# hansungkim98122/IGT-MPC-INT

Measured on NVIDIA B200. Metric: converged MPC solves/sec, higher is better.
Workload: dtype f64

## Files before the change

### igt_mpc_int_b200/csrc/igt_abi.cu

```cuda
#include <cuda_runtime.h>
#include <cstdio>
#include <cstdlib>
#include <cstring>
#include <string>
#include <vector>
#include <new>
#include <mutex>

#include "../../include/igt_mpc.h"
#include "solver_core.cuh"
#include "params_host.hpp"
#include "mlp_tc.cuh"

using namespace igt;

#ifndef SOLVE_BLOCK
#define SOLVE_BLOCK 256
#endif
#define SLOTS_PER_SM SOLVE_BLOCK

constexpr int N_CSLOTS = 8;
__constant__ DevParams<float> c_Pf[N_CSLOTS];
__constant__ DevParams<double> c_Pd[N_CSLOTS];
static_assert(N_CSLOTS * (sizeof(DevParams<float>) + sizeof(DevParams<double>)) <= 60 * 1024, "constant memory budget");

template <> struct igt::ConstP<float> { static __device__ __forceinline__ const DevParams<float> &get(int s) { return c_Pf[s]; } };
template <> struct igt::ConstP<double> { static __device__ __forceinline__ const DevParams<double> &get(int s) { return c_Pd[s]; } };
#include "episode.cuh"

template <typename T, bool OBCA>
__global__ void __launch_bounds__(128) guess_kernel(ProbIO io, long B, double *guess, int cs)
{
    long p = (long)blockIdx.x * blockDim.x + threadIdx.x;
    if (p >= B) return;
    if (io.u_init && (!io.warm || io.warm[p])) return;
    const DevParams<T> &P = ConstP<T>::get(cs);
    Solver<T, Ws<T, 32, OBCA>> sv(P);
    sv.compute_guess(io, p, guess + p * P.N * 2);
}

#ifndef IGT_RSTG
#define IGT_RSTG 1
#endif
template <typename T, bool TC, bool OBCA, bool COOP = false, bool BANK = false>
__global__ void __launch_bounds__(SOLVE_BLOCK, 1) solve_kernel(typename std::conditional<BANK, ProbIONet<T>, ProbIO>::type io, T *ws, long n_slots, long B, Sched sc,
                                                               const double *guess, T *mlp_scratch, int mlp_width,
                                                               MlpTcWeights wt, int quota, int cs)
{
    extern __shared__ __align__(16) uint8_t dyn_smem[];
    long slot = (long)blockIdx.x * blockDim.x + threadIdx.x;
    const DevParams<T> &P = ConstP<T>::get(cs);
    MlpTcCtx tc;
    if (TC) mlp_tc_setup(tc, dyn_smem, wt);
    constexpr bool RSTG = IGT_RSTG && !TC && !COOP;
    solve_persistent<T, TC, 32, OBCA, COOP, RSTG, BANK>(P, io, ws, slot, B, sc, guess,
                            mlp_scratch ? mlp_scratch + slot * 12 * (long)mlp_width : nullptr, mlp_width, &tc, quota, cs, dyn_smem,
                            RSTG ? dyn_smem + (COOP ? mlp_coop_smem_bytes<T>(SOLVE_BLOCK) : 0) : nullptr);
    if (TC) mlp_tc_teardown(tc);
}

template <typename T, bool OBCA>
__global__ void __launch_bounds__(SOLVE_BLOCK, 1) solve_small_kernel(ProbIO io, long B, Sched sc, const double *guess, int cs)
{
    extern __shared__ __align__(16) uint8_t dyn_smem[];
    const DevParams<T> &P = ConstP<T>::get(cs);
    solve_persistent<T, false, 1, OBCA>(P, io, reinterpret_cast<T *>(dyn_smem), 0, B, sc, guess, (T *)nullptr, 0, nullptr, 1, cs);
}

__global__ void __launch_bounds__(128) rollout_kernel(int B, const float *__restrict__ z0,
                                                      const float *__restrict__ U,
                                                      const float *__restrict__ curv_, float *__restrict__ Z,
                                                      float *__restrict__ A, float *__restrict__ Bm, int cs)
{
    int p = blockIdx.x * blockDim.x + threadIdx.x;
    if (p >= B) return;
    const DevParams<float> &P = c_Pf[cs];
    const int N = P.N;
    float z[NZ], comp[NZ], curv[3] = { curv_[3 * p], curv_[3 * p + 1], curv_[3 * p + 2] };
#pragma unroll
    for (int i = 0; i < NZ; i++) { z[i] = z0[(long)p * NZ + i]; comp[i] = 0.f; Z[(long)p * (N + 1) * NZ + i] = z[i]; }
    const float h = P.h;
    for (int k = 0; k < N; k++) {
        float u[2] = { U[((long)p * N + k) * 2], U[((long)p * N + k) * 2 + 1] };
        if (A) {
            float zn[NZ], Sc[NSENS], S[NZ][NSEED];
            rk4_step_sens(P, z, u, curv, zn, Sc);
            expand_sens(P, Sc, S);
            float *Ak = A + ((long)p * N + k) * NZ * NZ, *Bk = Bm + ((long)p * N + k) * NZ * 2;
#pragma unroll
            for (int i = 0; i < NZ; i++) {
#pragma unroll
                for (int j = 0; j < NZ; j++) Ak[i * NZ + j] = (i == j && j < 3) ? 1.f : 0.f;
                Ak[i * NZ + IEY] = S[i][0]; Ak[i * NZ + IEPSI] = S[i][1]; Ak[i * NZ + IV] = S[i][2]; Ak[i * NZ + IPSI] = S[i][3];
                Bk[i * 2] = S[i][4]; Bk[i * 2 + 1] = S[i][5];
            }
        }
        const StepK<float> c = step_setup(P, z, u, curv);
        const double b0d = curv[0], b1d = curv[1];
        auto Kof = [&](double sd) { return (sd >= b0d ? curv[2] : 0.f) - (sd >= b1d ? curv[2] : 0.f); };
        for (int it = 0; it < P.n_rk; it++) {
            Deriv<float> k1, k2, k3, k4;
            RhsJac<float> J;
            const float hh = 0.5f * h;
            const double sd = (double)z[IS] - (double)comp[IS];
            stage_deriv<float, false, true>(c, z[IS], z[IEY], z[IEPSI], z[IV], z[IPSI], k1, J, Kof(sd));
            stage_deriv<float, false, true>(c, z[IS] + hh * k1.s, z[IEY] + hh * k1.ey, z[IEPSI] + hh * k1.ep, z[IV] + hh * u[0],
                                            z[IPSI] + hh * k1.ps, k2, J, Kof(sd + (double)hh * (double)k1.s));
            stage_deriv<float, false, true>(c, z[IS] + hh * k2.s, z[IEY] + hh * k2.ey, z[IEPSI] + hh * k2.ep, z[IV] + hh * u[0],
                                            z[IPSI] + hh * k2.ps, k3, J, Kof(sd + (double)hh * (double)k2.s));
            stage_deriv<float, false, true>(c, z[IS] + h * k3.s, z[IEY] + h * k3.ey, z[IEPSI] + h * k3.ep, z[IV] + h * u[0],
                                            z[IPSI] + hh * k3.ps, k4, J, Kof(sd + (double)h * (double)k3.s));
            float inc[NZ];
            inc[IX] = h / 6.f * (k1.x + 2.f * k2.x + 2.f * k3.x + k4.x);
            inc[IY] = h / 6.f * (k1.y + 2.f * k2.y + 2.f * k3.y + k4.y);
            inc[IS] = h / 6.f * (k1.s + 2.f * k2.s + 2.f * k3.s + k4.s);
            inc[IEY] = h / 6.f * (k1.ey + 2.f * k2.ey + 2.f * k3.ey + k4.ey);
            inc[IEPSI] = h / 6.f * (k1.ep + 2.f * k2.ep + 2.f * k3.ep + k4.ep);
            inc[IV] = h * u[0];
            inc[IPSI] = h / 6.f * (k1.ps + 2.f * k2.ps + 2.f * k3.ps + k4.ps);
// ... 112 lines not shown
                                                      const MlpNet<double> *nets)
{
    long p = (long)blockIdx.x * blockDim.x + threadIdx.x;
    if (p >= B) return;
    const DevParams<double> &P = c_Pd[cs];
    TermVal<double> t;
    double cx[4] = { ctx[4 * p], ctx[4 * p + 1], ctx[4 * p + 2], ctx[4 * p + 3] };
    double *sc = scratch + p * 12 * (long)width;
    if (BANK) mlp_eval_thread_net(nets[net_idx[p]], sN[p], vN[p], cx, sc, sc + 6 * width, width, t, true);
    else mlp_eval_thread(P, sN[p], vN[p], cx, sc, sc + 6 * width, width, t, true);
    out[6 * p] = t.V; out[6 * p + 1] = t.gs; out[6 * p + 2] = t.gv; out[6 * p + 3] = t.Hss; out[6 * p + 4] = t.Hsv; out[6 * p + 5] = t.Hvv;
}

template <bool BANK>
__global__ void __launch_bounds__(256, 1) mlp_coop_kernel(long B, const double *sN, const double *vN, const double *ctx,
                                                          double *out, int cs, const int *net_idx, const MlpNet<double> *nets)
{
    extern __shared__ __align__(16) uint8_t dyn_smem[];
    const DevParams<double> &P = c_Pd[cs];
    for (long base = (long)blockIdx.x * 256; base < B; base += (long)gridDim.x * 256) {
        const long p = base + threadIdx.x;
        const bool valid = p < B;
        double cx[4] = { 0, 0, 0, 0 }, o[6], s = 0, v = 0;
        int net = 0;
        if (valid) { s = sN[p]; v = vN[p]; for (int i = 0; i < 4; i++) cx[i] = ctx[4 * p + i]; if (BANK) net = net_idx[p]; }
        if (BANK) mlp_coop_eval_bank(nets, dyn_smem, valid, net, s, v, cx, o);
        else mlp_coop_eval(P, dyn_smem, valid, s, v, cx, o);
        if (valid) for (int i = 0; i < 6; i++) out[6 * p + i] = o[i];
    }
}

template <typename T>
__global__ void __launch_bounds__(256) fma_peak_kernel(T *out, int iters)
{
    T a0 = T(threadIdx.x) * T(1e-3), a1 = a0 + T(1), a2 = a0 + T(2), a3 = a0 + T(3);
    T a4 = a0 + T(4), a5 = a0 + T(5), a6 = a0 + T(6), a7 = a0 + T(7);
    const T m = T(0.999999), c = T(1e-6);
    for (int i = 0; i < iters; i++) {
        a0 = a0 * m + c; a1 = a1 * m + c; a2 = a2 * m + c; a3 = a3 * m + c;
        a4 = a4 * m + c; a5 = a5 * m + c; a6 = a6 * m + c; a7 = a7 * m + c;
    }
    out[(long)blockIdx.x * blockDim.x + threadIdx.x] = a0 + a1 + a2 + a3 + a4 + a5 + a6 + a7;
}

struct igt_handle {
    igt_params prm;
    DevParams<float> Pf;
    DevParams<double> Pd;
    bool has_mlp = false;
    MlpTcWeights tc = {};
    int use_tc = 0;
    bool coop_ok = false;
    int use_small = 1;
    int mlp_width = 0;
    std::vector<void *> mlp_bufs[MAX_MLP_NETS];
    MlpNet<double> netd[MAX_MLP_NETS] = {};
    MlpNet<float> netf[MAX_MLP_NETS] = {};
    int net_width[MAX_MLP_NETS] = {};
    void *bank = nullptr;
    void *ws = nullptr; size_t ws_bytes = 0;
    void *mlp_scratch = nullptr; size_t mlp_scratch_bytes = 0;
    void *stage = nullptr; size_t stage_bytes = 0;
    void *guess = nullptr; size_t guess_bytes = 0;
    void *episode = nullptr; size_t episode_bytes = 0;
    int n_sm = 0;
    long long launches = 0;
    std::string err;
    int device = 0;
    std::mutex mu;
    cudaStream_t hstream = nullptr;
    void *pin = nullptr; size_t pin_bytes = 0;
    cudaEvent_t last_use = nullptr;
    cudaStream_t last_stream = nullptr;
    bool used = false;
    unsigned long long version[2] = { 1, 1 };
    int cslot[2] = { -1, -1 };
};

struct CSlot { const igt_handle *owner = nullptr; unsigned long long version = 0; cudaEvent_t ev = nullptr; };
constexpr int MAX_DEV = 16;
static std::mutex g_slot_mu;
static CSlot g_slots[MAX_DEV][2][N_CSLOTS];
static unsigned g_slot_rr[MAX_DEV][2];

static std::string g_create_err;
static_assert(IGT_MAX_MLP_NETS == MAX_MLP_NETS, "bank size");

#define CK(call)                                                                                   \
    do {                                                                                           \
        cudaError_t _e = (call);                                                                   \
        if (_e != cudaSuccess) {                                                                   \
            h->err = std::string(#call) + ": " + cudaGetErrorString(_e);                           \
            return IGT_ECUDA;                                                                      \
        }                                                                                          \
    } while (0)

static int grow(igt_handle *h, void **buf, size_t *have, size_t need, cudaStream_t st)
{
    if (*have >= need) return IGT_OK;
    if (*buf) { CK(cudaFreeAsync(*buf, st)); *buf = nullptr; *have = 0; }
    CK(cudaMallocAsync(buf, need, st));
    *have = need;
    return IGT_OK;
}

static int begin_call(igt_handle *h, cudaStream_t st)
// ... 314 lines not shown
    const bool f64 = h->prm.precision == IGT_PREC_F64, obca = obs_psi != nullptr;
    if (obca && !f64) { h->err = "igt_solve: the OBCA collision rows (obs_psi) need precision f64"; return IGT_EINVAL; }
    if (B == 0) return IGT_OK;
    int rc = begin_call(h, st), cs = 0;
    if (rc) return rc;
    WsLayout L; L.init(h->prm.N, h->prm.n_cinf, obca ? NGE_OBCA : NGE, obca ? NHE_OBCA : NHE);
    size_t esz = f64 ? 8 : 4;
    const size_t small_smem = (size_t)L.total * esz;
    const bool small = h->use_small && !nn_ctx && B <= h->n_sm && small_smem <= 200 * 1024;
    const int bs = SOLVE_BLOCK;
    long n_cta = ((long)B + 31) / 32;
    if (n_cta > h->n_sm) n_cta = h->n_sm;
    long per_cta = ((long)B + n_cta - 1) / n_cta;
    int quota = (int)((per_cta + 31) / 32 * 32);
    if (quota > bs) quota = bs;
    long n_slots = n_cta * bs;
    rc = small ? IGT_OK : grow(h, &h->ws, &h->ws_bytes, (size_t)L.total * n_slots * esz, st);
    if (rc) return rc;
    const bool use_tc = nn_ctx && !bank && h->tc.enabled && h->use_tc && !obca;
    const int width = bank ? bank_width(h) : h->mlp_width;
    const bool use_coop = nn_ctx && !use_tc && f64 && (bank ? width <= MLP_COOP_W : h->coop_ok) && !obca;
    if (nn_ctx && !use_tc && !use_coop) {
        rc = grow(h, &h->mlp_scratch, &h->mlp_scratch_bytes, (size_t)12 * width * n_slots * esz, st);
        if (rc) return rc;
    }
    const size_t off_guess = 256;
    rc = grow(h, &h->guess, &h->guess_bytes, off_guess + (size_t)B * h->prm.N * 2 * sizeof(double), st);
    if (rc) return rc;
    char *sb = (char *)h->guess;
    Sched sc;
    sc.counter = (unsigned long long *)sb;
    double *guess = (double *)(sb + off_guess);
    rc = acquire_cslot(h, f64 ? 1 : 0, st, &cs);
    if (rc) return rc;
    CK(cudaMemsetAsync(sb, 0, 256, st));
    ProbIO io = { x0, u_prev, curv, obs_xy, nn_ctx, u_init, x, u, cost, viol, status, iters };
    io.obs_psi = obs_psi;
    io.warm = warm;
    ProbIONet<double> iob;
    static_cast<ProbIO &>(iob) = io;
    iob.net_idx = net_idx;
    iob.nets = (const MlpNet<double> *)h->bank;
    if (!u_init || warm) {
        int gbs = 128, ggs = (B + gbs - 1) / gbs;
        if (obca) guess_kernel<double, true><<<ggs, gbs, 0, st>>>(io, B, guess, cs);
        else if (f64) guess_kernel<double, false><<<ggs, gbs, 0, st>>>(io, B, guess, cs);
        else guess_kernel<float, false><<<ggs, gbs, 0, st>>>(io, B, guess, cs);
        h->launches++;
    }
    int gs = (int)(n_slots / bs);
    if (small) {
        if (obca) {
            CK(cudaFuncSetAttribute(solve_small_kernel<double, true>, cudaFuncAttributeMaxDynamicSharedMemorySize, (int)small_smem));
            solve_small_kernel<double, true><<<B, bs, small_smem, st>>>(io, B, sc, guess, cs);
        } else if (f64) {
            CK(cudaFuncSetAttribute(solve_small_kernel<double, false>, cudaFuncAttributeMaxDynamicSharedMemorySize, (int)small_smem));
            solve_small_kernel<double, false><<<B, bs, small_smem, st>>>(io, B, sc, guess, cs);
        } else {
            CK(cudaFuncSetAttribute(solve_small_kernel<float, false>, cudaFuncAttributeMaxDynamicSharedMemorySize, (int)small_smem));
            solve_small_kernel<float, false><<<B, bs, small_smem, st>>>(io, B, sc, guess, cs);
        }
    } else if (bank) {
        double *scr = (double *)h->mlp_scratch;
        const int rsm = IGT_RSTG ? RSTG_SLOTS * SOLVE_BLOCK * (int)esz : 0;
        if (use_coop) {
            const int sm = mlp_coop_bank_smem_bytes<double>(SOLVE_BLOCK);
            CK(cudaFuncSetAttribute(solve_kernel<double, false, false, true, true>, cudaFuncAttributeMaxDynamicSharedMemorySize, sm));
            solve_kernel<double, false, false, true, true><<<gs, bs, sm, st>>>(iob, (double *)h->ws, n_slots, B, sc, guess, nullptr, width, h->tc, quota, cs);
        } else if (obca) {
            CK(cudaFuncSetAttribute(solve_kernel<double, false, true, false, true>, cudaFuncAttributeMaxDynamicSharedMemorySize, rsm));
            solve_kernel<double, false, true, false, true><<<gs, bs, rsm, st>>>(iob, (double *)h->ws, n_slots, B, sc, guess, scr, width, h->tc, quota, cs);
        } else if (f64) {
            CK(cudaFuncSetAttribute(solve_kernel<double, false, false, false, true>, cudaFuncAttributeMaxDynamicSharedMemorySize, rsm));
            solve_kernel<double, false, false, false, true><<<gs, bs, rsm, st>>>(iob, (double *)h->ws, n_slots, B, sc, guess, scr, width, h->tc, quota, cs);
        } else {
            CK(cudaFuncSetAttribute(solve_kernel<float, false, false, false, true>, cudaFuncAttributeMaxDynamicSharedMemorySize, rsm));
            solve_kernel<float, false, false, false, true><<<gs, bs, rsm, st>>>(iob_f32(iob, h), (float *)h->ws, n_slots, B, sc, guess, (float *)h->mlp_scratch, width, h->tc, quota, cs);
        }
    } else if (use_tc) {
        if (f64) {
            CK(cudaFuncSetAttribute(solve_kernel<double, true, false>, cudaFuncAttributeMaxDynamicSharedMemorySize, TC_SMEM_BYTES));
            solve_kernel<double, true, false><<<gs, bs, TC_SMEM_BYTES, st>>>(io, (double *)h->ws, n_slots, B, sc, guess, nullptr, h->mlp_width, h->tc, quota, cs);
        } else {
            CK(cudaFuncSetAttribute(solve_kernel<float, true, false>, cudaFuncAttributeMaxDynamicSharedMemorySize, TC_SMEM_BYTES));
            solve_kernel<float, true, false><<<gs, bs, TC_SMEM_BYTES, st>>>(io, (float *)h->ws, n_slots, B, sc, guess, nullptr, h->mlp_width, h->tc, quota, cs);
        }
    } else if (use_coop) {
        const int sm = mlp_coop_smem_bytes<double>(SOLVE_BLOCK);
        CK(cudaFuncSetAttribute(solve_kernel<double, false, false, true>, cudaFuncAttributeMaxDynamicSharedMemorySize, sm));
        solve_kernel<double, false, false, true><<<gs, bs, sm, st>>>(io, (double *)h->ws, n_slots, B, sc, guess, nullptr, h->mlp_width, h->tc, quota, cs);
    } else if (obca) {
        const int rsm = IGT_RSTG ? RSTG_SLOTS * SOLVE_BLOCK * 8 : 0;
        CK(cudaFuncSetAttribute(solve_kernel<double, false, true>, cudaFuncAttributeMaxDynamicSharedMemorySize, rsm));
        solve_kernel<double, false, true><<<gs, bs, rsm, st>>>(io, (double *)h->ws, n_slots, B, sc, guess,
                                                               nn_ctx ? (double *)h->mlp_scratch : nullptr, h->mlp_width, h->tc, quota, cs);
    } else if (f64) {
        const int rsm = IGT_RSTG ? RSTG_SLOTS * SOLVE_BLOCK * 8 : 0;
        CK(cudaFuncSetAttribute(solve_kernel<double, false, false>, cudaFuncAttributeMaxDynamicSharedMemorySize, rsm));
        solve_kernel<double, false, false><<<gs, bs, rsm, st>>>(io, (double *)h->ws, n_slots, B, sc, guess,
                                                                nn_ctx ? (double *)h->mlp_scratch : nullptr, h->mlp_width, h->tc, quota, cs);
    } else {
        const int rsm = IGT_RSTG ? RSTG_SLOTS * SOLVE_BLOCK * 4 : 0;
        CK(cudaFuncSetAttribute(solve_kernel<float, false, false>, cudaFuncAttributeMaxDynamicSharedMemorySize, rsm));
        solve_kernel<float, false, false><<<gs, bs, rsm, st>>>(io, (float *)h->ws, n_slots, B, sc, guess,
                                                               nn_ctx ? (float *)h->mlp_scratch : nullptr, h->mlp_width, h->tc, quota, cs);
    }
    h->launches++;
    CK(cudaGetLastError());
    return end_call(h, st, f64 ? 2 : 1);
}

int igt_solve_ex_dev(igt_handle *h, int B, const double *x0, const double *u_prev, const double *curv,
                     const double *obs_xy, const double *obs_psi, const double *nn_ctx, const int *net_idx, const double *u_init,
                     double *x, double *u, double *cost, double *viol, int *status, int *iters, void *stream)
{
    if (!h) return IGT_EINVAL;
    std::lock_guard<std::mutex> lk(h->mu);
    return solve_dev_impl(h, B, x0, u_prev, curv, obs_xy, obs_psi, nn_ctx, u_init, x, u, cost, viol, status, iters,
                          (cudaStream_t)stream, nullptr, net_idx);
}

int igt_solve_dev(igt_handle *h, int B, const double *x0, const double *u_prev, const double *curv,
                  const double *obs_xy, const double *obs_psi, const double *nn_ctx, const double *u_init, double *x,
                  double *u, double *cost, double *viol, int *status, int *iters, void *stream)
{
    return igt_solve_ex_dev(h, B, x0, u_prev, curv, obs_xy, obs_psi, nn_ctx, nullptr, u_init, x, u, cost, viol, status, iters, stream);
}

int igt_solve_ex_host(igt_handle *h, int B, const double *x0, const double *u_prev, const double *curv,
                      const double *obs_xy, const double *obs_psi, const double *nn_ctx, const int *net_idx, const double *u_init,
                      double *x, double *u, double *cost, double *viol, int *status, int *iters)
{
    if (!h) return IGT_EINVAL;
    if (B < 0 || !x0 || !u_prev || !curv || !obs_xy || !x || !u || !cost || !viol || !status || !iters) {
        h->err = "igt_solve: null argument"; return IGT_EINVAL;
    }
    if (net_idx && !nn_ctx) { h->err = "igt_solve: net_idx needs nn_ctx (gt_mpc)"; return IGT_EINVAL; }
    if (B == 0) return IGT_OK;
    std::lock_guard<std::mutex> lk(h->mu);
    if (net_idx) { const int rc0 = check_net_idx(h, B, net_idx, "igt_solve"); if (rc0) return rc0; }
    CK(cudaSetDevice(h->device));
    if (!h->hstream) CK(cudaStreamCreateWithFlags(&h->hstream, cudaStreamNonBlocking));
    cudaStream_t st = h->hstream;
    int rc = begin_call(h, st);
    if (rc) return rc;
    const int N = h->prm.N;
    size_t nb = (size_t)B;
    size_t n_x0 = nb * 7, n_up = nb * 2, n_c = nb * 3, n_o = nb * (N + 1) * 2, n_ctx = nn_ctx ? nb * 4 : 0;
    size_t n_ui = u_init ? nb * N * 2 : 0, n_x = nb * (N + 1) * 7, n_u = nb * N * 2, n_op = obs_psi ? nb * (N + 1) : 0;
    size_t n_in = n_x0 + n_up + n_c + n_o + n_ctx + n_ui + n_op, n_out = n_x + n_u + 2 * nb;
    size_t in_bytes = n_in * 8, out_bytes = n_out * 8 + 2 * nb * 4, total = in_bytes + out_bytes;
    rc = grow(h, &h->stage, &h->stage_bytes, total + (net_idx ? nb * 4 : 0), st);
    if (rc) return rc;
    int *dnet = (int *)((char *)h->stage + total);
    if (net_idx) CK(cudaMemcpyAsync(dnet, net_idx, nb * 4, cudaMemcpyHostToDevice, st));
    double *d = (double *)h->stage;
    double *dx0 = d, *dup = dx0 + n_x0, *dc = dup + n_up, *dob = dc + n_c, *dctx = dob + n_o, *dui = dctx + n_ctx;
    double *dop = dui + n_ui;
// ... 313 lines not shown
        CK(cudaMemcpyAsync(dnet, veh_net.data(), nb * 4, cudaMemcpyHostToDevice, st));
    }
    CK(cudaMemcpyAsync(eb.z, z0, n_z * 8, cudaMemcpyHostToDevice, st));
    CK(cudaMemcpyAsync(eb.u_prev, u_prev0, n_up * 8, cudaMemcpyHostToDevice, st));
    CK(cudaMemcpyAsync(dcv, curv, n_cv * 8, cudaMemcpyHostToDevice, st));
    CK(cudaMemcpyAsync(drd, route_desc, n_rd * 8, cudaMemcpyHostToDevice, st));
    CK(cudaMemcpyAsync(den, enc, n_en * 8, cudaMemcpyHostToDevice, st));
    CK(cudaMemsetAsync(eb.prev_ok, 0, nb * 4, st));
    CK(cudaMemcpy2DAsync(eb.z_cl, (size_t)(T + 1) * 7 * 8, eb.z, 7 * 8, 7 * 8, nb, cudaMemcpyDeviceToDevice, st));
    std::vector<cudaEvent_t> ev;
    if (step_ms) { ev.resize(T + 1); for (auto &e : ev) CK(cudaEventCreate(&e)); CK(cudaEventRecord(ev[0], st)); }
    const int bs = 128, gs = (B + bs - 1) / bs;
    int cs = 0;
    for (int t = 0; t < T; t++) {
        const int cur = t & 1, prv = cur ^ 1;
        if (obca) episode_pre_kernel<true><<<gs, bs, 0, st>>>(eb, B, N, h->prm.dt, t, gt_mpc, px[prv], pu[prv]);
        else episode_pre_kernel<false><<<gs, bs, 0, st>>>(eb, B, N, h->prm.dt, t, gt_mpc, px[prv], pu[prv]);
        h->launches++;
        rc = solve_dev_impl(h, B, eb.z, eb.u_prev, eb.curv, eb.obs, eb.obs_psi, gt_mpc ? eb.ctx : nullptr, eb.u_init, px[cur], pu[cur],
                            pcost[cur], pviol[cur], pst[cur], pit[cur], st, eb.warm, dnet);
        if (rc) return rc;
        rc = acquire_cslot(h, 1, st, &cs);
        if (rc) return rc;
        episode_post_kernel<<<gs, bs, 0, st>>>(eb, B, N, T, t, h->prm.a_min, px[cur], pu[cur], pst[cur], cs);
        h->launches++;
        if (step_ms) CK(cudaEventRecord(ev[t + 1], st));
    }
    CK(cudaGetLastError());
    CK(cudaMemcpyAsync(z_cl, eb.z_cl, n_zcl * 8, cudaMemcpyDeviceToHost, st));
    CK(cudaMemcpyAsync(u_cl, eb.u_cl, n_ucl * 8, cudaMemcpyDeviceToHost, st));
    CK(cudaMemcpyAsync(solved, eb.solved, nb * T * 4, cudaMemcpyDeviceToHost, st));
    rc = end_call(h, st, 2);
    if (rc) return rc;
    CK(cudaStreamSynchronize(st));
    if (step_ms) {
        for (int t = 0; t < T; t++) CK(cudaEventElapsedTime(&step_ms[t], ev[t], ev[t + 1]));
        for (auto &e : ev) cudaEventDestroy(e);
    }
    return IGT_OK;
}

int igt_episode_run_host(igt_handle *h, int E, int steps, int mode, const double *route_desc, const double *curv,
                         const double *z0, const double *u_prev0, const double *enc, double *z_cl, double *u_cl,
                         int *solved, float *step_ms)
{
    return igt_episode_run_ex_host(h, E, steps, mode, route_desc, curv, z0, u_prev0, enc, nullptr, z_cl, u_cl, solved, step_ms);
}

int igt_set_option(igt_handle *h, const char *name, double value)
{
    if (!h || !name) return IGT_EINVAL;
    if (strcmp(name, "tensor_core_mlp") == 0) { h->use_tc = value != 0.0; return IGT_OK; }
    if (strcmp(name, "latency_path") == 0) { h->use_small = value != 0.0; return IGT_OK; }
    h->err = std::string("igt_set_option: unknown option ") + name;
    return IGT_EINVAL;
}

}
```

### igt_mpc_int_b200/csrc/solver_core.cuh

```cuda
#pragma once
#include <cmath>
#include <cstdint>
#include <type_traits>
#include "mlp_tc.cuh"
#include "obca.cuh"

#ifdef __CUDACC__
#define IGT_HD __host__ __device__ __forceinline__
#define IGT_HDN __host__ __device__ __noinline__
#else
#define IGT_HD inline
#define IGT_HDN
#endif

#ifndef IGT_PF_DIST
#define IGT_PF_DIST 1
#endif
#ifndef IGT_PF_DIST_R
#define IGT_PF_DIST_R 1
#endif

namespace igt {

constexpr int NZ = 7, NA = 9, NW = 11, NSEED = 6;
// ... 1339 lines not shown
                T F[NA][NW];
                load_F(P, w, k, F);
#pragma unroll
                for (int i = 0; i < NA; i++) {
                    T acc = T(0);
#pragma unroll
                    for (int j = 0; j < NW; j++) if (fmask(i, j)) acc += F[i][j] * dw[j];
                    dz[i] = acc;
                }
            }
            visit_rows<false, W::obca>(P, k, z, up, u, ox(k), oy(k), opsi(k), [&](auto SL, int, T c, auto I0, T g0, auto I1, T g1, auto I2, T g2, T, T, T) {
                constexpr int sl = decltype(SL)::value, i0 = decltype(I0)::value, i1 = decltype(I1)::value, i2 = decltype(I2)::value;
                const T y = yv[sl];
                T dc = g0 * dw[i0];
                if constexpr (i1 >= 0) dc += g1 * dw[i1];
                if constexpr (i2 >= 0) dc += g2 * dw[i2];
                T dy = -(c + y) - dc;
                const T ty = tau * y;
                const bool tighter = dy < T(0) && -dy * an > ty * ad;
                an = tighter ? ty : an; ad = tighter ? -dy : ad;
            });
            if (k == N - 1) {
#pragma unroll 1
                for (int m0 = 0; m0 < P.n_cinf; m0 += 8) {
                    T y8[8];
#pragma unroll
                    for (int j = 0; j < 8; j++) if (m0 + j < P.n_cinf) y8[j] = w.Y(b, o + NSLOT + m0 + j);
#pragma unroll
                    for (int j = 0; j < 8; j++)
                        if (m0 + j < P.n_cinf) {
                            const T A0 = P.cinf_A[m0 + j][0], A1 = P.cinf_A[m0 + j][1], y = y8[j];
                            const T c = A0 * z[IV] + A1 * u[0] - P.cinf_b[m0 + j];
                            T dc = A0 * dw[IV];
                            dc += A1 * dw[IUA];
                            T dy = -(c + y) - dc;
                            const T ty = tau * y;
                            const bool tighter = dy < T(0) && -dy * an > ty * ad;
                            an = tighter ? ty : an; ad = tighter ? -dy : ad;
                        }
                }
            }
        }
        alpha = (an / ad) * P.alpha_safety;
    }

    IGT_HD bool backward_pre()
    {
        const bool fresh = need_back == 2;
        if (fresh) { adjoint_sweep(); need_back = 1; }
        test_and_update();
        return fresh && !done;
    }

    IGT_HD void backward_post()
    {
        for (;;) {
            if (riccati_sweep()) break;
            reg = fmax(fmax(reg * P.reg_up, P.reg_min), reg_hint);
            if (reg > P.reg_max) { status = acceptable() ? 6 : 3; done = true; return; }
        }
        need_back = 0;
        ls = 0;
        step_bound();
    }

    IGT_HD void backward()
    {
        if (need_back == 2) {
            const NodeCtx<T> c = node_ctx();
            for (int k = 0; k <= P.N; k++) node_phase1(P, w, c, k);
        }
        if (backward_pre()) {
            const NodeCtx<T> c = node_ctx();
            for (int k = 0; k <= P.N; k++) node_phase2(P, w, c, k);
        }
        if (!done) backward_post();
    }

    IGT_HD void collect_trial(int j)
    {
        const int nb = cand_buf(cur, j);
        trial_ok = w.Tc(nb, 0) != T(0);
        if (!trial_ok) return;
        T th = T(0), lg = T(0), bad = T(0);
#if !defined(IGT_COLLECT_BATCH)
        for (int k = 0; k <= P.N; k++) { th += w.Tr(nb, k, 0); lg += w.Tr(nb, k, 1); bad += w.Tr(nb, k, 2); }
#else
        for (int k0 = 0; k0 <= P.N; k0 += 8) {
            T t8[8][3];
#pragma unroll
            for (int i = 0; i < 8; i++)
                if (k0 + i <= P.N) { t8[i][0] = w.Tr(nb, k0 + i, 0); t8[i][1] = w.Tr(nb, k0 + i, 1); t8[i][2] = w.Tr(nb, k0 + i, 2); }
#pragma unroll
            for (int i = 0; i < 8; i++)
                if (k0 + i <= P.N) { th += t8[i][0]; lg += t8[i][1]; bad += t8[i][2]; }
        }
#endif
        Jcand = w.Tc(nb, 1); thetacand = th; lgcand = lg;
        if (bad > T(0)) trial_ok = false;
    }

    IGT_HD bool trial_passes() const
    {
        if (!trial_ok) return false;
        T phin = Jcand - tcand.V - mu * lgcand;
        return (phin == phin) && fabs(phin) < T(1e30) &&
               (phin < phi - P.eps_phi * fabs(phi) || thetacand < thetacur * (T(1) - P.gamma_theta) ||
                (thetacand <= P.theta_small && phin <= phi + fmax(P.eps_phi * fmax(T(1), fabs(phi)), phi_noise)));
    }

    IGT_HD void finish_trials(int jacc, int tried)
    {
        if (jacc >= 0) {
            cur = cand_buf(cur, jacc);
            Jcur = Jcand; lgcur = lgcand; thetacur = thetacand; tcur = tcand;
            reg = reg > P.reg_min ? reg / P.reg_down : T(0);
// ... 128 lines not shown
    NodeCtx<T> ctx[MAX_SOLVE_BLOCK];
};

template <typename T, typename S>
__device__ __forceinline__ int cta_list_build(bool need, long bound, const S &sv, NodeList<T> &nl, int *my_idx = nullptr)
{
    const unsigned FULL = 0xffffffffu;
    const int tid = threadIdx.x, lane = tid & 31, warp = tid >> 5, nw = blockDim.x >> 5;
    const unsigned m = __ballot_sync(FULL, need);
    if (lane == 0) nl.wcnt[warp] = __popc(m);
    __syncthreads();
    int base = 0, n = 0;
    for (int i = 0; i < nw; i++) { int c = nl.wcnt[i]; if (i < warp) base += c; n += c; }
    if (need) {
        const int idx = base + __popc(m & ((1u << lane) - 1u));
        nl.slot[idx] = (int)bound;
        nl.ctx[idx] = sv.node_ctx();
        if (my_idx) *my_idx = idx;
    }
    __syncthreads();
    return n;
}

template <typename T> struct ConstP;

template <typename T, int PHASE, int STRIDE, bool OBCA, bool RSTG, bool BANK>
__device__ __noinline__ void phase_items(T *ws_base, const NodeList<T> *nl, int n, int n_spec)
{
    const DevParams<T> &P = ConstP<T>::get(nl->cslot);
    Ws<T, STRIDE, OBCA, RSTG && PHASE != 3> w; w.init_layout(P.N, P.n_cinf);
    if (RSTG && PHASE != 3) { w.rs = reinterpret_cast<T *>(nl->rstg) + threadIdx.x; w.rs_stride = blockDim.x; }
    if (PHASE == 1 || PHASE == 2) {
        const int total = n * (P.N + 1);
        for (int it = threadIdx.x; it < total; it += blockDim.x) {
            const int j = it % n, k = it / n;
            w.bind(ws_base, nl->slot[j]);
            if (PHASE == 1) node_phase1(P, w, nl->ctx[j], k);
            else node_phase2(P, w, nl->ctx[j], k);
        }
    } else if (PHASE == 3) {
        for (int it = threadIdx.x; it < n * n_spec; it += blockDim.x) {
            const int q = it % n, j = it / n;
            if (j < P.n_alpha - nl->ctx[q].ls) { w.bind(ws_base, nl->slot[q]); rollout_item(P, w, nl->ctx[q], j); }
        }
    } else {
        const int total = n * n_spec * (P.N + 1);
        for (int it = threadIdx.x; it < total; it += blockDim.x) {
            const int q = it % n, r = it / n, j = r % n_spec, k = r / n_spec;
            if (j < P.n_alpha - nl->ctx[q].ls) { w.bind(ws_base, nl->slot[q]); node_phase3(P, w, nl->ctx[q], k, j); }
        }
    }
}

template <typename T, int PHASE, int STRIDE, bool RSTG, typename S>
__device__ __forceinline__ void node_phase_cta(const DevParams<T> &P, T *ws_base, const WsLayout &L, bool need,
                                               long bound, const S &sv, NodeList<T> &nl)
{
    const int n = cta_list_build(need, bound, sv, nl);
    if (n > 0) phase_items<T, PHASE, STRIDE, S::obca, RSTG, S::bank>(ws_base, &nl, n, 1);
    __syncthreads();
}

#ifdef IGT_PHASE_CLOCKS
__device__ long long g_mid_t;
#define IGT_MID_TICK() do { if (blockIdx.x == 0 && threadIdx.x == 0) g_mid_t = clock64(); } while (0)
#else
#define IGT_MID_TICK() do { } while (0)
#endif

#ifndef IGT_SPEC_BUDGET
#define IGT_SPEC_BUDGET IGT_MAX_SOLVE_BLOCK
#endif
template <typename T, int STRIDE, bool RSTG, typename S>
__device__ __forceinline__ int trial_phase_cta(const DevParams<T> &P, T *ws_base, const WsLayout &L, bool need,
                                               long bound, const S &sv, NodeList<T> &nl, bool speculate, int &n_out,
                                               int *my_idx = nullptr)
{
    const int n = cta_list_build(need, bound, sv, nl, my_idx);
    n_out = n;
    if (n == 0) { IGT_MID_TICK(); return 1; }
    int n_spec = 1;
    if (speculate) { n_spec = IGT_SPEC_BUDGET / n; n_spec = n_spec < 1 ? 1 : (n_spec > P.n_alpha ? P.n_alpha : n_spec); }
    phase_items<T, 3, STRIDE, S::obca, false, S::bank>(ws_base, &nl, n, n_spec);
    __syncthreads();
    IGT_MID_TICK();
    phase_items<T, 4, STRIDE, S::obca, RSTG, S::bank>(ws_base, &nl, n, n_spec);
    __syncthreads();
    return n_spec;
}

template <typename T, bool COOP, bool BANK, typename WS>
__device__ __forceinline__ void tc_candidates(const DevParams<T> &P, const ProbIO &io, T *ws_base, const WS &wproto,
                                              const NodeList<T> &nl, int n, int n_spec, MlpTcCtx *tc, uint8_t *coop_smem,
                                              int jlo = 0, bool filter = false)
{
    if (n == 0) return;
    const int t = threadIdx.x, q = t % n, j = jlo + t / n;
    bool valid = j < n_spec && j < P.n_alpha - nl.ctx[q].ls && (!filter || nl.more[q]);
    WS w = wproto;
    int nb = 0;
    using V = typename std::conditional<COOP, T, float>::type;
    V cx[4] = { V(0), V(0), V(0), V(0) }, o[6], sN = V(0), vN = V(0);
    int net = 0;
    if (valid) {
        w.bind(ws_base, nl.slot[q]);
        nb = cand_buf(nl.ctx[q].cur, j);
        valid = w.Tc(nb, 0) != T(0);
    }
    if (valid) {
        const long p = (nl.ctx[q].x0p - io.x0) / NZ;
#pragma unroll
        for (int i = 0; i < 4; i++) cx[i] = V(io.ctx[p * 4 + i]);
        sN = V(w.Z(nb, P.N, IS)); vN = V(w.Z(nb, P.N, IV));
        if (BANK) net = bank_io<T>(io).net_idx[p];
    }
    if (__syncthreads_or(valid)) {
        if constexpr (COOP && BANK) mlp_coop_eval_bank(bank_io<T>(io).nets, coop_smem, valid, net, sN, vN, cx, o);
        else if constexpr (COOP) mlp_coop_eval(P, coop_smem, valid, sN, vN, cx, o);
        else mlp_tc_eval(*tc, valid, sN, vN, cx, o);
        if (valid) {
#pragma unroll
            for (int i = 0; i < 6; i++) w.Tc(nb, 2 + i) = T(o[i]);
        }
    }
    __syncthreads();
}

#ifdef IGT_PHASE_CLOCKS
__device__ long long g_phase_clk[16];
__device__ long long g_round_clk[512];
__device__ int g_round_n[512];
__device__ int g_round_ph[512][12];
__device__ long long g_cta_clk[512];
__device__ int g_cta_rounds[512];
__device__ int g_round_mx[512][4];
#define IGT_TICK(i) do { if (clk_on) { long long t_ = clock64(); clk[i] += t_ - clk_t; if (round_i < 512) g_round_ph[round_i][i] += (int)((t_ - clk_t) >> 10); clk_t = t_; } } while (0)
#else
#define IGT_TICK(i) do { } while (0)
#endif

template <typename T, bool TC, int STRIDE = 32, bool OBCA = false, bool COOP = false, bool RSTG = false, bool BANK = false>
__device__ __forceinline__ void solve_persistent(const DevParams<T> &P, const ProbIO &io, T *ws_base,
                                                 long slot, long B, const Sched &sc,
                                                 const double *guess, T *mlp_scratch, int mlp_width, MlpTcCtx *tc,
                                                 int quota, int cslot, uint8_t *coop_smem = nullptr, void *rstg_smem = nullptr)
{
    __shared__ NodeList<T> nl;
    if (threadIdx.x == 0) { nl.cslot = cslot; nl.rstg = rstg_smem; }
    static_assert(!(TC && BANK), "the tensor-core value term holds one network");
    Solver<T, Ws<T, STRIDE, OBCA>, BANK> sv(P);
    sv.w.init_layout(P.N, P.n_cinf);
    sv.w.bind(ws_base, slot);
    sv.mlp_scratch = mlp_scratch; sv.mlp_width = mlp_width;
    const unsigned FULL = 0xffffffffu;
    bool active = false, exhausted = (int)threadIdx.x >= quota;
    long p = -1;
    const long bound = slot;
    if (TC) sv.phi_noise = T(3e-7);
    constexpr bool CTA_MLP = TC || COOP;
#ifdef IGT_PHASE_CLOCKS
    const bool clk_on = blockIdx.x == 0 && threadIdx.x == 0;
    long long clk[16] = { 0 }, clk_t = clock64(), round_t = clk_t;
    const long long cta_t0 = clk_t;
    int round_i = 0, cta_rounds = 0;
    if (clk_on) for (int i = 0; i < 12; i++) g_round_ph[0][i] = 0;
#endif
    for (;;) {
        bool fresh = false;
        if (!active && !exhausted) {
            p = (long)atomicAdd(sc.counter, 1ULL);
            if (p >= B) exhausted = true;
            else {
                const bool warm = io.u_init && (!io.warm || io.warm[p]);
                const double *u_src = (warm ? io.u_init : guess) + p * P.N * 2;
                if (sv.init(io, p, io.ctx != nullptr, u_src, warm)) {
                    if (!CTA_MLP) sv.terminal_of(sv.cur, sv.tcur, true);
                    active = true;
                    fresh = true;
                } else {
                    sv.write_out(io, p);
                }
            }
        }
        if (TC) {
            if (__syncthreads_or(fresh)) {
                float cx[4] = { float(sv.ctx[0]), float(sv.ctx[1]), float(sv.ctx[2]), float(sv.ctx[3]) }, o[6];
                float sN = fresh ? float(sv.w.Z(sv.cur, P.N, IS)) : 0.f, vN = fresh ? float(sv.w.Z(sv.cur, P.N, IV)) : 0.f;
                mlp_tc_eval(*tc, fresh, sN, vN, cx, o);
                if (fresh) term_from_tc(o, sv.tcur);
            }
        }
        if (COOP) {
            const bool want = fresh && sv.gt;
            if (__syncthreads_or(want)) {
                T o[6];
                const T sN = want ? sv.w.Z(sv.cur, P.N, IS) : T(0), vN = want ? sv.w.Z(sv.cur, P.N, IV) : T(0);
                if constexpr (BANK) mlp_coop_eval_bank(bank_io<T>(io).nets, coop_smem, want, want ? bank_io<T>(io).net_idx[p] : 0, sN, vN, sv.ctx, o);
                else mlp_coop_eval(P, coop_smem, want, sN, vN, sv.ctx, o);
                if (want) { sv.tcur.V = o[0]; sv.tcur.gs = o[1]; sv.tcur.gv = o[2]; sv.tcur.Hss = o[3]; sv.tcur.Hsv = o[4]; sv.tcur.Hvv = o[5]; }
            }
        }
        const bool wants_exit = __all_sync(FULL, exhausted && !active);
#ifdef IGT_PHASE_CLOCKS
        cta_rounds++;
        const int cta_busy = __syncthreads_count(active);
        if (clk_on && round_i < 512) {
            long long t_ = clock64();
            g_round_clk[round_i] = t_ - round_t; g_round_n[round_i] = cta_busy; round_t = t_; round_i++;
            if (round_i < 512) for (int i = 0; i < 12; i++) g_round_ph[round_i][i] = 0;
        }
#else
        const int cta_busy = __syncthreads_or(active);
#endif
        if (__syncthreads_and(wants_exit)) break;
        if (!cta_busy) { IGT_TICK(9); continue; }
        IGT_TICK(0);
        const bool back = active && sv.need_back;
        node_phase_cta<T, 1, STRIDE, RSTG>(P, ws_base, sv.w.L, back && sv.need_back == 2, bound, sv, nl);
        IGT_TICK(1);
#ifdef IGT_PHASE_CLOCKS
        __shared__ int s_round_i;
        if (clk_on) s_round_i = round_i;
        __syncthreads();
        const int rnd_ = s_round_i;
        const long long ta_ = clock64();
#endif
        const bool p2 = back && sv.backward_pre();
#ifdef IGT_PHASE_CLOCKS
        if (blockIdx.x == 0 && back && rnd_ < 512) atomicMax(&g_round_mx[rnd_][0], (int)((clock64() - ta_) >> 10));
#endif
        IGT_TICK(2);
        node_phase_cta<T, 2, STRIDE, RSTG>(P, ws_base, sv.w.L, p2, bound, sv, nl);
        IGT_TICK(3);
        if (back && !sv.done) {
#ifdef IGT_PHASE_CLOCKS
            const long long tr_ = clock64();
            int nsw_ = 0;
            for (;;) {
                nsw_++;
                if (sv.riccati_sweep()) break;
                sv.reg = fmax(fmax(sv.reg * P.reg_up, P.reg_min), sv.reg_hint);
                if (sv.reg > P.reg_max) { sv.status = sv.acceptable() ? 6 : 3; sv.done = true; break; }
            }
            const long long ts_ = clock64();
            IGT_TICK(4);
            if (!sv.done) { sv.need_back = 0; sv.ls = 0; sv.step_bound(); }
            if (blockIdx.x == 0 && rnd_ < 512) {
                atomicMax(&g_round_mx[rnd_][1], (int)((ts_ - tr_) >> 10));
                atomicMax(&g_round_mx[rnd_][2], (int)((clock64() - ts_) >> 10));
                atomicMax(&g_round_mx[rnd_][3], nsw_);
            }
            IGT_TICK(5);
#else
            sv.backward_post();
#endif
        }
        __syncthreads();
        IGT_TICK(6);
        const bool trying = active && !sv.done;
        int n_try = 0;
        int my_idx = 0;
        const int n_spec = trial_phase_cta<T, STRIDE, RSTG>(P, ws_base, sv.w.L, trying, bound, sv, nl, true, n_try, &my_idx);
#ifdef IGT_PHASE_CLOCKS
        if (clk_on) { long long m_ = g_mid_t; clk[7] += m_ - clk_t; if (round_i < 512) g_round_ph[round_i][7] += (int)((m_ - clk_t) >> 10); clk_t = m_; }
#endif
        IGT_TICK(11);
        if (CTA_MLP) {
            const int left = P.n_alpha - sv.ls, nj = n_spec < left ? n_spec : left;
            tc_candidates<T, COOP, BANK>(P, io, ws_base, sv.w, nl, n_try, 1, tc, coop_smem);
            int tried = 0, jacc = -1;
            if (trying) jacc = sv.judge_trials(0, 1, true, tried);
            const bool more = trying && jacc < 0 && nj > 1;
            if (trying) nl.more[my_idx] = more ? 1 : 0;
            if (__syncthreads_or(more)) {
                tc_candidates<T, COOP, BANK>(P, io, ws_base, sv.w, nl, n_try, n_spec, tc, coop_smem, 1, true);
                if (more) jacc = sv.judge_trials(1, nj, true, tried);
            }
            if (trying) sv.finish_trials(jacc, tried);
        } else if (trying) {
            const int left = P.n_alpha - sv.ls;
            sv.accept_trials(n_spec < left ? n_spec : left, false);
        }
        IGT_TICK(8);
        if (active && sv.done) { sv.write_out(io, p); active = false; }
        IGT_TICK(10);
    }
#ifdef IGT_PHASE_CLOCKS
// ... 11 lines not shown
```

Baseline: 304,100.

## Compute step bound cooperatively per warp when few slots need backward pass

When few threads in a CTA need the post-Riccati step-bound computation (counted with __syncthreads_count), each such slot's fraction-to-boundary search is handed to a whole warp. Operands are distributed across lanes and broadcast with shuffles, instead of each thread running it serially. This targets tail latency in rounds where most slots are idle and a few long serial step_bound calls hold up the CTA. It adds a CTA-wide barrier and count every round, plus a new option coop_sweep_max that defaults to 32.

```diff
diff --git a/igt_mpc_int_b200/csrc/igt_abi.cu b/igt_mpc_int_b200/csrc/igt_abi.cu
--- a/igt_mpc_int_b200/csrc/igt_abi.cu
+++ b/igt_mpc_int_b200/csrc/igt_abi.cu
@@ -45,7 +45,7 @@
 template <typename T, bool TC, bool OBCA, bool COOP = false, bool BANK = false>
 __global__ void __launch_bounds__(SOLVE_BLOCK, 1) solve_kernel(typename std::conditional<BANK, ProbIONet<T>, ProbIO>::type io, T *ws, long n_slots, long B, Sched sc,
                                                                const double *guess, T *mlp_scratch, int mlp_width,
-                                                               MlpTcWeights wt, int quota, int cs)
+                                                               MlpTcWeights wt, int quota, int cs, int coop)
 {
     extern __shared__ __align__(16) uint8_t dyn_smem[];
     long slot = (long)blockIdx.x * blockDim.x + threadIdx.x;
@@ -54,17 +54,17 @@
     if (TC) mlp_tc_setup(tc, dyn_smem, wt);
     constexpr bool RSTG = IGT_RSTG && !TC && !COOP;
     solve_persistent<T, TC, 32, OBCA, COOP, RSTG, BANK>(P, io, ws, slot, B, sc, guess,
-                            mlp_scratch ? mlp_scratch + slot * 12 * (long)mlp_width : nullptr, mlp_width, &tc, quota, cs, dyn_smem,
+                            mlp_scratch ? mlp_scratch + slot * 12 * (long)mlp_width : nullptr, mlp_width, &tc, quota, cs, coop, dyn_smem,
                             RSTG ? dyn_smem + (COOP ? mlp_coop_smem_bytes<T>(SOLVE_BLOCK) : 0) : nullptr);
     if (TC) mlp_tc_teardown(tc);
 }
 
 template <typename T, bool OBCA>
-__global__ void __launch_bounds__(SOLVE_BLOCK, 1) solve_small_kernel(ProbIO io, long B, Sched sc, const double *guess, int cs)
+__global__ void __launch_bounds__(SOLVE_BLOCK, 1) solve_small_kernel(ProbIO io, long B, Sched sc, const double *guess, int cs, int coop)
 {
     extern __shared__ __align__(16) uint8_t dyn_smem[];
     const DevParams<T> &P = ConstP<T>::get(cs);
-    solve_persistent<T, false, 1, OBCA>(P, io, reinterpret_cast<T *>(dyn_smem), 0, B, sc, guess, (T *)nullptr, 0, nullptr, 1, cs);
+    solve_persistent<T, false, 1, OBCA>(P, io, reinterpret_cast<T *>(dyn_smem), 0, B, sc, guess, (T *)nullptr, 0, nullptr, 1, cs, coop);
 }
 
 __global__ void __launch_bounds__(128) rollout_kernel(int B, const float *__restrict__ z0,
@@ -283,6 +283,7 @@
     int use_tc = 0;
     bool coop_ok = false;
     int use_small = 1;
+    int coop_sweep_max = 32;
     int mlp_width = 0;
     std::vector<void *> mlp_bufs[MAX_MLP_NETS];
     MlpNet<double> netd[MAX_MLP_NETS] = {};
@@ -703,13 +704,13 @@
     if (small) {
         if (obca) {
             CK(cudaFuncSetAttribute(solve_small_kernel<double, true>, cudaFuncAttributeMaxDynamicSharedMemorySize, (int)small_smem));
-            solve_small_kernel<double, true><<<B, bs, small_smem, st>>>(io, B, sc, guess, cs);
+            solve_small_kernel<double, true><<<B, bs, small_smem, st>>>(io, B, sc, guess, cs, h->coop_sweep_max);
         } else if (f64) {
             CK(cudaFuncSetAttribute(solve_small_kernel<double, false>, cudaFuncAttributeMaxDynamicSharedMemorySize, (int)small_smem));
-            solve_small_kernel<double, false><<<B, bs, small_smem, st>>>(io, B, sc, guess, cs);
+            solve_small_kernel<double, false><<<B, bs, small_smem, st>>>(io, B, sc, guess, cs, h->coop_sweep_max);
         } else {
             CK(cudaFuncSetAttribute(solve_small_kernel<float, false>, cudaFuncAttributeMaxDynamicSharedMemorySize, (int)small_smem));
-            solve_small_kernel<float, false><<<B, bs, small_smem, st>>>(io, B, sc, guess, cs);
+            solve_small_kernel<float, false><<<B, bs, small_smem, st>>>(io, B, sc, guess, cs, h->coop_sweep_max);
         }
     } else if (bank) {
         double *scr = (double *)h->mlp_scratch;
@@ -717,44 +718,44 @@
         if (use_coop) {
             const int sm = mlp_coop_bank_smem_bytes<double>(SOLVE_BLOCK);
             CK(cudaFuncSetAttribute(solve_kernel<double, false, false, true, true>, cudaFuncAttributeMaxDynamicSharedMemorySize, sm));
-            solve_kernel<double, false, false, true, true><<<gs, bs, sm, st>>>(iob, (double *)h->ws, n_slots, B, sc, guess, nullptr, width, h->tc, quota, cs);
+            solve_kernel<double, false, false, true, true><<<gs, bs, sm, st>>>(iob, (double *)h->ws, n_slots, B, sc, guess, nullptr, width, h->tc, quota, cs, h->coop_sweep_max);
         } else if (obca) {
             CK(cudaFuncSetAttribute(solve_kernel<double, false, true, false, true>, cudaFuncAttributeMaxDynamicSharedMemorySize, rsm));
-            solve_kernel<double, false, true, false, true><<<gs, bs, rsm, st>>>(iob, (double *)h->ws, n_slots, B, sc, guess, scr, width, h->tc, quota, cs);
+            solve_kernel<double, false, true, false, true><<<gs, bs, rsm, st>>>(iob, (double *)h->ws, n_slots, B, sc, guess, scr, width, h->tc, quota, cs, h->coop_sweep_max);
         } else if (f64) {
             CK(cudaFuncSetAttribute(solve_kernel<double, false, false, false, true>, cudaFuncAttributeMaxDynamicSharedMemorySize, rsm));
-            solve_kernel<double, false, false, false, true><<<gs, bs, rsm, st>>>(iob, (double *)h->ws, n_slots, B, sc, guess, scr, width, h->tc, quota, cs);
+            solve_kernel<double, false, false, false, true><<<gs, bs, rsm, st>>>(iob, (double *)h->ws, n_slots, B, sc, guess, scr, width, h->tc, quota, cs, h->coop_sweep_max);
         } else {
             CK(cudaFuncSetAttribute(solve_kernel<float, false, false, false, true>, cudaFuncAttributeMaxDynamicSharedMemorySize, rsm));
-            solve_kernel<float, false, false, false, true><<<gs, bs, rsm, st>>>(iob_f32(iob, h), (float *)h->ws, n_slots, B, sc, guess, (float *)h->mlp_scratch, width, h->tc, quota, cs);
+            solve_kernel<float, false, false, false, true><<<gs, bs, rsm, st>>>(iob_f32(iob, h), (float *)h->ws, n_slots, B, sc, guess, (float *)h->mlp_scratch, width, h->tc, quota, cs, h->coop_sweep_max);
         }
     } else if (use_tc) {
         if (f64) {
             CK(cudaFuncSetAttribute(solve_kernel<double, true, false>, cudaFuncAttributeMaxDynamicSharedMemorySize, TC_SMEM_BYTES));
-            solve_kernel<double, true, false><<<gs, bs, TC_SMEM_BYTES, st>>>(io, (double *)h->ws, n_slots, B, sc, guess, nullptr, h->mlp_width, h->tc, quota, cs);
+            solve_kernel<double, true, false><<<gs, bs, TC_SMEM_BYTES, st>>>(io, (double *)h->ws, n_slots, B, sc, guess, nullptr, h->mlp_width, h->tc, quota, cs, h->coop_sweep_max);
         } else {
             CK(cudaFuncSetAttribute(solve_kernel<float, true, false>, cudaFuncAttributeMaxDynamicSharedMemorySize, TC_SMEM_BYTES));
-            solve_kernel<float, true, false><<<gs, bs, TC_SMEM_BYTES, st>>>(io, (float *)h->ws, n_slots, B, sc, guess, nullptr, h->mlp_width, h->tc, quota, cs);
+            solve_kernel<float, true, false><<<gs, bs, TC_SMEM_BYTES, st>>>(io, (float *)h->ws, n_slots, B, sc, guess, nullptr, h->mlp_width, h->tc, quota, cs, h->coop_sweep_max);
         }
     } else if (use_coop) {
         const int sm = mlp_coop_smem_bytes<double>(SOLVE_BLOCK);
         CK(cudaFuncSetAttribute(solve_kernel<double, false, false, true>, cudaFuncAttributeMaxDynamicSharedMemorySize, sm));
-        solve_kernel<double, false, false, true><<<gs, bs, sm, st>>>(io, (double *)h->ws, n_slots, B, sc, guess, nullptr, h->mlp_width, h->tc, quota, cs);
+        solve_kernel<double, false, false, true><<<gs, bs, sm, st>>>(io, (double *)h->ws, n_slots, B, sc, guess, nullptr, h->mlp_width, h->tc, quota, cs, h->coop_sweep_max);
     } else if (obca) {
         const int rsm = IGT_RSTG ? RSTG_SLOTS * SOLVE_BLOCK * 8 : 0;
         CK(cudaFuncSetAttribute(solve_kernel<double, false, true>, cudaFuncAttributeMaxDynamicSharedMemorySize, rsm));
         solve_kernel<double, false, true><<<gs, bs, rsm, st>>>(io, (double *)h->ws, n_slots, B, sc, guess,
-                                                               nn_ctx ? (double *)h->mlp_scratch : nullptr, h->mlp_width, h->tc, quota, cs);
+                                                               nn_ctx ? (double *)h->mlp_scratch : nullptr, h->mlp_width, h->tc, quota, cs, h->coop_sweep_max);
     } else if (f64) {
         const int rsm = IGT_RSTG ? RSTG_SLOTS * SOLVE_BLOCK * 8 : 0;
         CK(cudaFuncSetAttribute(solve_kernel<double, false, false>, cudaFuncAttributeMaxDynamicSharedMemorySize, rsm));
         solve_kernel<double, false, false><<<gs, bs, rsm, st>>>(io, (double *)h->ws, n_slots, B, sc, guess,
-                                                                nn_ctx ? (double *)h->mlp_scratch : nullptr, h->mlp_width, h->tc, quota, cs);
+                                                                nn_ctx ? (double *)h->mlp_scratch : nullptr, h->mlp_width, h->tc, quota, cs, h->coop_sweep_max);
     } else {
         const int rsm = IGT_RSTG ? RSTG_SLOTS * SOLVE_BLOCK * 4 : 0;
         CK(cudaFuncSetAttribute(solve_kernel<float, false, false>, cudaFuncAttributeMaxDynamicSharedMemorySize, rsm));
         solve_kernel<float, false, false><<<gs, bs, rsm, st>>>(io, (float *)h->ws, n_slots, B, sc, guess,
-                                                               nn_ctx ? (float *)h->mlp_scratch : nullptr, h->mlp_width, h->tc, quota, cs);
+                                                               nn_ctx ? (float *)h->mlp_scratch : nullptr, h->mlp_width, h->tc, quota, cs, h->coop_sweep_max);
     }
     h->launches++;
     CK(cudaGetLastError());
@@ -1174,6 +1175,11 @@
     if (!h || !name) return IGT_EINVAL;
     if (strcmp(name, "tensor_core_mlp") == 0) { h->use_tc = value != 0.0; return IGT_OK; }
     if (strcmp(name, "latency_path") == 0) { h->use_small = value != 0.0; return IGT_OK; }
+    if (strcmp(name, "coop_sweep_max") == 0) {
+        if (!(value >= 0.0 && value <= 1e9)) { h->err = "igt_set_option: coop_sweep_max must be >= 0"; return IGT_EINVAL; }
+        h->coop_sweep_max = (int)value;
+        return IGT_OK;
+    }
     h->err = std::string("igt_set_option: unknown option ") + name;
     return IGT_EINVAL;
 }
diff --git a/igt_mpc_int_b200/csrc/solver_core.cuh b/igt_mpc_int_b200/csrc/solver_core.cuh
--- a/igt_mpc_int_b200/csrc/solver_core.cuh
+++ b/igt_mpc_int_b200/csrc/solver_core.cuh
@@ -1415,16 +1415,21 @@
         return fresh && !done;
     }
 
-    IGT_HD void backward_post()
+    IGT_HD bool riccati_post()
     {
         for (;;) {
             if (riccati_sweep()) break;
             reg = fmax(fmax(reg * P.reg_up, P.reg_min), reg_hint);
-            if (reg > P.reg_max) { status = acceptable() ? 6 : 3; done = true; return; }
+            if (reg > P.reg_max) { status = acceptable() ? 6 : 3; done = true; return false; }
         }
         need_back = 0;
         ls = 0;
-        step_bound();
+        return true;
+    }
+
+    IGT_HD void backward_post()
+    {
+        if (riccati_post()) step_bound();
     }
 
     IGT_HD void backward()
@@ -1659,6 +1664,128 @@
     }
 }
 
+constexpr int BOUND_OPS = 72;
+template <typename T, typename W>
+__device__ __forceinline__ T bound_op(const DevParams<T> &P, const W &w, const NodeCtx<T> &c, int k, int i)
+{
+    const int N = P.N, b = c.cur;
+    if (k > N || i >= BOUND_OPS) return T(0);
+    if (i < NSLOT) return slot_used(N, k, i) ? w.Y(b, row_off(N, P.n_cinf, k) + i - slot_base(N, k)) : T(0);
+    i -= NSLOT;
+    if (i < NZ) return w.Z(b, k, i);
+    i -= NZ;
+    if (i < 2) return k == 0 ? c.uprev[i] : w.U(b, k - 1, i);
+    i -= 2;
+    if (i < 2) return T(c.obs[2 * k + i]);
+    i -= 2;
+    if (k == N) return T(0);
+    if (i < 2) return w.U(b, k, i);
+    i -= 2;
+    if (i < 2) return w.ku(k, i);
+    i -= 2;
+    if (i < 2 * NA) return w.KK(k, i / NA, i % NA);
+    return w.Sens(k, i - 2 * NA);
+}
+enum { BO_Z = NSLOT, BO_UP = BO_Z + NZ, BO_OBS = BO_UP + 2, BO_U = BO_OBS + 2, BO_KU = BO_U + 2, BO_KK = BO_KU + 2,
+       BO_SENS = BO_KK + 2 * NA };
+static_assert(BO_SENS + NSENS == BOUND_OPS, "bound operand table");
+template <typename T>
+struct ShflOps {
+    const T *v;
+    __device__ __forceinline__ T op(int i) const { return __shfl_sync(0xffffffffu, v[i >> 5], i & 31); }
+    __device__ __forceinline__ T Sens(int, int e) const { return op(BO_SENS + e); }
+};
+
+template <typename T, int STRIDE, bool BANK>
+__device__ __noinline__ void bound_items(T *ws_base, NodeList<T> *nl, int n)
+{
+    const DevParams<T> &P = ConstP<T>::get(nl->cslot);
+    Ws<T, STRIDE> w; w.init_layout(P.N, P.n_cinf);
+    const int N = P.N, lane = threadIdx.x & 31, nw = blockDim.x >> 5;
+    constexpr int NV = (BOUND_OPS + 31) / 32;
+    for (int q = threadIdx.x >> 5; q < n; q += nw) {
+        w.bind(ws_base, nl->slot[q]);
+        const NodeCtx<T> c = nl->ctx[q];
+        const int b = c.cur;
+        const T tau = fmax(P.tau_min, T(1) - c.mu);
+        T an = T(1), ad = T(1), dz[NA];
+#pragma unroll
+        for (int i = 0; i < NA; i++) dz[i] = T(0);
+        T nv[NV];
+#pragma unroll
+        for (int j = 0; j < NV; j++) nv[j] = bound_op(P, w, c, 0, lane + 32 * j);
+        for (int k = 0; k <= N; k++) {
+            T v[NV];
+#pragma unroll
+            for (int j = 0; j < NV; j++) { v[j] = nv[j]; nv[j] = bound_op(P, w, c, k + 1, lane + 32 * j); }
+            const ShflOps<T> so{ v };
+            T z[NZ], up[2], u[2] = { T(0), T(0) }, dw[NW], yv[NSLOT];
+#pragma unroll
+            for (int sl = 0; sl < NSLOT; sl++) yv[sl] = so.op(sl);
+#pragma unroll
+            for (int i = 0; i < NZ; i++) z[i] = so.op(BO_Z + i);
+            up[0] = so.op(BO_UP); up[1] = so.op(BO_UP + 1);
+            const T ox = so.op(BO_OBS), oy = so.op(BO_OBS + 1);
+#pragma unroll
+            for (int i = 0; i < NA; i++) dw[i] = dz[i];
+            dw[IUA] = T(0); dw[IUD] = T(0);
+            if (k < N) {
+                u[0] = so.op(BO_U); u[1] = so.op(BO_U + 1);
+                T d0 = so.op(BO_KU), d1 = so.op(BO_KU + 1);
+#pragma unroll
+                for (int j = 0; j < NA; j++) { d0 += so.op(BO_KK + j) * dz[j]; d1 += so.op(BO_KK + NA + j) * dz[j]; }
+                dw[IUA] = d0; dw[IUD] = d1;
+                T F[NA][NW];
+                load_F(P, so, k, F);
+#pragma unroll
+                for (int i = 0; i < NA; i++) {
+                    T acc = T(0);
+#pragma unroll
+                    for (int j = 0; j < NW; j++) if (fmask(i, j)) acc += F[i][j] * dw[j];
+                    dz[i] = acc;
+                }
+            }
+            visit_rows<false, false>(P, k, z, up, u, ox, oy, T(0), [&](auto SL, int, T cv, auto I0, T g0, auto I1, T g1, auto I2, T g2, T, T, T) {
+                constexpr int sl = decltype(SL)::value, i0 = decltype(I0)::value, i1 = decltype(I1)::value, i2 = decltype(I2)::value;
+                const T y = yv[sl];
+                T dc = g0 * dw[i0];
+                if constexpr (i1 >= 0) dc += g1 * dw[i1];
+                if constexpr (i2 >= 0) dc += g2 * dw[i2];
+                T dy = -(cv + y) - dc;
+                const T ty = tau * y;
+                const bool tighter = dy < T(0) && -dy * an > ty * ad;
+                an = tighter ? ty : an; ad = tighter ? -dy : ad;
+            });
+            if (k == N - 1) {
+                const int o = row_off(N, P.n_cinf, k);
+                T yc[MAX_CINF / 32];
+#pragma unroll
+                for (int j = 0; j < MAX_CINF / 32; j++) {
+                    const int m = lane + 32 * j;
+                    yc[j] = m < P.n_cinf ? w.Y(b, o + NSLOT + m) : T(0);
+                }
+#pragma unroll
+                for (int j = 0; j < MAX_CINF / 32; j++) {
+#pragma unroll 1
+                    for (int l = 0; l < 32; l++) {
+                        const int m = 32 * j + l;
+                        if (m >= P.n_cinf) break;
+                        const T A0 = P.cinf_A[m][0], A1 = P.cinf_A[m][1], y = __shfl_sync(0xffffffffu, yc[j], l);
+                        const T cv = A0 * z[IV] + A1 * u[0] - P.cinf_b[m];
+                        T dc = A0 * dw[IV];
+                        dc += A1 * dw[IUA];
+                        T dy = -(cv + y) - dc;
+                        const T ty = tau * y;
+                        const bool tighter = dy < T(0) && -dy * an > ty * ad;
+                        an = tighter ? ty : an; ad = tighter ? -dy : ad;
+                    }
+                }
+            }
+        }
+        if (lane == 0) nl->ctx[q].alpha = (an / ad) * P.alpha_safety;
+    }
+}
+
 template <typename T, int PHASE, int STRIDE, bool RSTG, typename S>
 __device__ __forceinline__ void node_phase_cta(const DevParams<T> &P, T *ws_base, const WsLayout &L, bool need,
                                                long bound, const S &sv, NodeList<T> &nl)
@@ -1750,7 +1877,8 @@
 __device__ __forceinline__ void solve_persistent(const DevParams<T> &P, const ProbIO &io, T *ws_base,
                                                  long slot, long B, const Sched &sc,
                                                  const double *guess, T *mlp_scratch, int mlp_width, MlpTcCtx *tc,
-                                                 int quota, int cslot, uint8_t *coop_smem = nullptr, void *rstg_smem = nullptr)
+                                                 int quota, int cslot, int coop_max, uint8_t *coop_smem = nullptr,
+                                                 void *rstg_smem = nullptr)
 {
     __shared__ NodeList<T> nl;
     if (threadIdx.x == 0) { nl.cslot = cslot; nl.rstg = rstg_smem; }
@@ -1839,7 +1967,28 @@
         IGT_TICK(2);
         node_phase_cta<T, 2, STRIDE, RSTG>(P, ws_base, sv.w.L, p2, bound, sv, nl);
         IGT_TICK(3);
-        if (back && !sv.done) {
+        const bool post = back && !sv.done;
+        const int n_post = !OBCA && coop_max > 0 ? __syncthreads_count(post) : 0;
+        if (n_post > 0 && n_post <= coop_max) {
+#ifdef IGT_PHASE_CLOCKS
+            const long long tr_ = clock64();
+#endif
+            const bool bnd = post && sv.riccati_post();
+#ifdef IGT_PHASE_CLOCKS
+            const long long ts_ = clock64();
+            if (blockIdx.x == 0 && post && rnd_ < 512) atomicMax(&g_round_mx[rnd_][1], (int)((ts_ - tr_) >> 10));
+            IGT_TICK(4);
+#endif
+            int my_b = 0;
+            const int nb = cta_list_build(bnd, bound, sv, nl, &my_b);
+            if constexpr (!OBCA) { if (nb > 0) bound_items<T, STRIDE, BANK>(ws_base, &nl, nb); }
+            __syncthreads();
+            if (bnd) sv.alpha = nl.ctx[my_b].alpha;
+#ifdef IGT_PHASE_CLOCKS
+            if (blockIdx.x == 0 && bnd && rnd_ < 512) atomicMax(&g_round_mx[rnd_][2], (int)((clock64() - ts_) >> 10));
+            IGT_TICK(5);
+#endif
+        } else if (post) {
 #ifdef IGT_PHASE_CLOCKS
             const long long tr_ = clock64();
             int nsw_ = 0;
```

Result: no change. 302,300, median of 6 (-0.6%).
